# fmidev/RoadSurf

Hardware: AMD Instinct MI355X
Metric: point_timesteps_per_s (higher is better)
Workload: dtype f64

## Files before the change

### roadsurf_amd/csrc/rs_api.hip

```cpp
#include <hip/hip_runtime.h>
#include <atomic>
#include <cmath>
#include <cstdarg>
#include <cstdio>
#include <cstdlib>
#include <cstring>
#include <mutex>
#include <utility>
#include <vector>

#include "../../include/roadsurf.h"
#include "rs_kernels.h"
#include "rs_ens_table.hpp"
#include "rs_devutil.hpp"
#include <cstdint>
#include <algorithm>
#include "rs_consts_dev.h"
#include "rs_state.h"

static thread_local char g_err[512] = "";

static int set_err(const char *fmt, ...) {
  va_list ap;
  va_start(ap, fmt);
// ... 1266 lines not shown
  if (rs_read_div_mismatch(n, pl->stream) != hipSuccess) return -1;
  return which == 1 ? (int64_t)(n[1] + n[2]) : (int64_t)n[0];
}
int64_t rs_hip_div_mismatch_count(RsPlan *pl) { return div_mismatch(pl, 0); }
int64_t rs_hip_div_special_count(RsPlan *pl) { return div_mismatch(pl, 1); }
int rs_hip_div_samples(RsPlan *pl, double *out) {
  if (!pl || !out) return set_err("rs_hip_div_samples: bad arguments");
  HIP_OK(hipSetDevice(pl->device));
  HIP_OK(rs_read_div_samples(out, pl->stream));
  return 0;
}

int rs_hip_bl_stats(RsPlan *pl, int64_t *out) {
  if (!pl || !out) return set_err("rs_hip_bl_stats: bad arguments");
  HIP_OK(hipSetDevice(pl->device));
  unsigned long long v[56];
  HIP_OK(rs_read_bl_stats(v, pl->stream));
  for (int k = 0; k < 56; ++k) out[k] = (int64_t)v[k];
  return 0;
}

int rs_hip_division_mode(void) {
#if defined(RS_IEEE_DIV)
  return 0;
#elif defined(RS_DIV_CHECK)
  return 2;
#else
  return 1;
#endif
}

int rs_hip_test_math(RsPlan *pl, int32_t fn, int64_t n, const double *x, double *y) {
  if (!pl || !x || !y || n < 1 || fn < 0 || fn > 3) return set_err("rs_hip_test_math: bad arguments");
// ... 82 lines not shown
```

### roadsurf_amd/csrc/rs_consts_dev.h

```cpp
#pragma once
#include <cstdlib>
#include "../../include/roadsurf.h"

struct RsConstantsDev : RsConstants {
  double meltDen;
  double r_3600, r_3364, r_1000, r_IceMax, r_twoDT, r_DTSecs, r_meltDen, r_logUstar, r_logCond;
  int32_t bareFastOk;
  int32_t precFastOk;
  double chk[8];
  const double *relax_tab;
  const double *cpl_tab;
  double capDZF[RS_MAX_LAYERS + 2];
  double hs1F;
  double hcw[8];
  struct LayerRow {
    double capDZF, condDZ, DyC, dryCap, WCont, pad[3];
  } lk[RS_MAX_LAYERS + 2];
};

static inline void rs_consts_dev_fill(const RsConstants &c, RsConstantsDev &d) {
  static_cast<RsConstants &>(d) = c;
  d.meltDen = c.WatMHeat * c.WatDens;
  d.r_3600 = 1.0 / 3600.0;
  d.r_3364 = 1.0 / 3364.0;
  d.r_1000 = 1.0 / 1000.0;
  d.r_IceMax = 1.0 / 1.5;
  d.r_twoDT = 1.0 / c.twoDT;
  d.r_DTSecs = 1.0 / c.DTSecs;
  d.r_meltDen = 1.0 / d.meltDen;
  d.r_logUstar = 1.0 / c.logUstar;
  d.r_logCond = 1.0 / c.logCond;
  const float chk[8] = {100.0f, -0.1f, -90.0f, 120.0f, -1.0f, 4000.0f, 1000.0f, 500.0f};
  for (int i = 0; i < 8; ++i) d.chk[i] = (double)chk[i];
// ... 13 lines not shown
  }
  for (int j = 0; j < RS_MAX_LAYERS + 2; ++j) d.capDZF[j] = 0.0;
  d.hs1F = 0.0;
  for (int j = 1; j <= c.NLayers && j <= RS_MAX_LAYERS; ++j) {
    const volatile double chwt = 920.0 * 2100.0;
    const volatile double wc = c.WCont[j] * chwt;
    const volatile double vsh = c.dryCap[j] + wc;
    const volatile double den = c.DyC[j] * vsh;
    d.capDZF[j] = -(1.0 / den);
    d.lk[j].capDZF = d.capDZF[j];
    if (j == 1) {
      const volatile double num = vsh * c.HSfac1;
      d.hs1F = num / c.twoDT;
    }
  }
  d.bareFastOk = (c.MaxWatmms >= 0.0 && c.MaxSnowmms >= 0.0 && c.MaxIcemms >= 0.0 && c.MaxDepmms >= 0.0) ? 1 : 0;
  d.precFastOk = (c.MinPrecmm >= 0.0) ? 1 : 0;
}

static inline const char *rs_consts_domain_error(const RsConstants &c) {
  const double lo = 1e-30, hi = 1e30;
  auto pos = [&](double x) { return x > lo && x < hi; };
  auto mag = [&](double x) { return (x > lo && x < hi) || (x < -lo && x > -hi); };
  if (!pos(c.DTSecs) || !pos(c.twoDT)) return "DTSecs";
  if (!mag(c.logUstar)) return "logUstar = log(ZRefW/ZMom)";
  if (!mag(c.logCond)) return "logCond = log(ZRefT/ZHeat)";
  if (!(c.logMom > -hi && c.logMom < hi) || !(c.logHeat > -hi && c.logHeat < hi)) return "logMom/logHeat";
  if (!pos(c.VK_Const)) return "VK_Const";
  if (!pos(c.LVap) || !pos(c.LFus)) return "LVap/LFus";
  if (!pos(c.WatMHeat * c.WatDens)) return "WatMHeat*WatDens";
// ... 28 lines not shown
```

### roadsurf_amd/csrc/rs_kernels.hip

```cpp
#include <hip/hip_runtime.h>
#include <cstdlib>
#include "rs_physics.hpp"
#include "rs_state.h"
#include "rs_synth.h"
#include "rs_kernels.h"

#ifndef RS_CPL_WAVES
#define RS_CPL_WAVES 2
#endif
#ifndef RS_REGIME_WINDOW
#define RS_REGIME_WINDOW 30
#endif

namespace rs {

constexpr int kBlock = RS_BLOCK;

typedef RsConstantsDev __attribute__((address_space(4))) ConstsAS;
template <class Args>
__device__ __forceinline__ const ConstsAS &consts_of(Args a) {
  return *(const ConstsAS *)a->consts;
}

template <int NL, int NREG>
// ... 587 lines not shown
#endif
template <bool SCORE, bool A32>
__global__ void __launch_bounds__(kBlock, 4) step_kernel_hybrid(const StepArgs a) {
  __shared__ double math_lds[RS_MATH_LDS_DOUBLES];
  __shared__ double prof_lds[(15 - RS_HYBRID_REG) * kBlock];
  step_lanes<HybridProfile<15, RS_HYBRID_REG>, true, false, SCORE, false, false, A32>(a, math_lds, prof_lds);
}

template <bool FULL, bool DIAG = false>
__global__ void __launch_bounds__(kBlock, 4) step_kernel_lds(const StepArgs a) {
  extern __shared__ double lds[];
  __shared__ double math_lds[RS_MATH_LDS_DOUBLES];
  step_lanes<LdsProfile, FULL, false, true, false, false, false, DIAG>(a, math_lds, lds);
}

enum { PR_TAIR = 0, PR_VZ, PR_RHZ, PR_RAIN, PR_SNOW, PR_AVC, PR_EAIR, PR_SW, PR_LW, PR_OBS, PR_LEAN = PR_OBS, PR_FULL = PR_OBS + 1 };
template <int NPREP>
struct DuoMailT {
  double v[2][2][64];
  uint32_t failed[64];
  double prep[2][NPREP][64];
  uint32_t prep_bad[2][64];
};

template <bool FULL, bool SKYG = false, class Mail>
__device__ __forceinline__ void duo_put_prep(Mail &mail, int buf, uint32_t lane, const ForcingPrep &q) {
  double (*w)[64] = mail.prep[buf];
  w[PR_TAIR][lane] = q.tair; w[PR_VZ][lane] = q.vz; w[PR_RHZ][lane] = q.rhz; w[PR_RAIN][lane] = q.rain;
  w[PR_SNOW][lane] = q.snow;
  w[PR_AVC][lane] = q.AirHCap * q.AirDens;
  w[PR_EAIR][lane] = q.EAir;
  if (!SKYG) {
    w[PR_SW][lane] = q.sw;
    w[PR_LW][lane] = q.lw;
  }
  if (FULL) w[PR_OBS][lane] = q.tsurfobs;
  mail.prep_bad[buf][lane] = (q.bad ? 1u : 0u) | (q.night ? 2u : 0u) | (q.bad_rw ? 8u : 0u);
}
template <bool FULL, bool SKYG = false, class C, class Mail>
__device__ __forceinline__ ForcingPrep duo_get_prep(const C &c, const Mail &mail, int buf, uint32_t lane,
                                                    const uint32_t *skyfl = nullptr) {
  const double (*w)[64] = mail.prep[buf];
  ForcingPrep q;
  q.tair = w[PR_TAIR][lane]; q.vz = w[PR_VZ][lane]; q.rhz = w[PR_RHZ][lane]; q.rain = w[PR_RAIN][lane];
  q.snow = w[PR_SNOW][lane];
  const double AirVCap = w[PR_AVC][lane];
  q.AirVCap = AirVCap;
  q.EAir = w[PR_EAIR][lane]; q.sw = w[PR_SW][lane]; q.lw = w[PR_LW][lane];
  if (FULL) q.tsurfobs = w[PR_OBS][lane];
  uint32_t flags = mail.prep_bad[buf][lane];
  if (SKYG) flags |= skyfl[buf * 64 + lane];
  {
    const double fricN = c.TrfFricNgt, fricD = c.TrFfricDay;
    q.night = (flags & 2u) != 0u;
    q.trffric = q.night ? fricN : fricD;
  }
  q.PsychC = R4(0.1) * (R4(0.00063) * (q.tair + R4(273.15)) + R4(0.47496));
  q.den0 = AirVCap * (q.tair + R4(273.15));
  q.vkvz = c.VK_Const * q.vz;
  q.avk = AirVCap * c.VK_Const;
  q.bad = (flags & 1u) != 0u;
  q.stop = SKYG && (flags & 4u) != 0u;
  q.bad_rw = (flags & 8u) != 0u;
  return q;
}

__device__ __forceinline__ void duo_meet() { asm volatile("s_waitcnt lgkmcnt(0)\n\ts_barrier" ::: "memory"); }

template <int NL, bool SCORE, bool FULL = false, bool SKY = false, bool SKYG = false, bool OUTIDX = false,
          bool CPL = false, bool REPLAY = false>
__device__ __forceinline__ void duo_surface(const MathTab &mt, DuoMailT<FULL ? PR_FULL : PR_LEAN> &mail, const StepArgs &a,
                                            const uint32_t *skyfl = nullptr) {
// ... 1355 lines not shown
```

### roadsurf_amd/csrc/rs_math.hpp

```cpp
#pragma once
#include <hip/hip_runtime.h>
#include "rs_glibc_tables.h"

namespace rs {

static __constant__ uint64_t c_gl_exp_tab[256] = {0};
static __constant__ uint64_t c_gl_log_tab[256] = {0};

enum { RS_K_EXP_SHIFT, RS_K_EXP_C2, RS_K_EXP_C4, RS_K_LOG_A1, RS_K_LOG_A3, RS_K_LOG_B1,
       RS_K_LOG_B4, RS_K_LOG_B7, RS_K_COUNT };
static __constant__ uint64_t c_gl_coef[RS_K_COUNT] = {
    RS_GL_EXP_SHIFT, RS_GL_EXP_C2, RS_GL_EXP_C4, RS_GL_LOG_A1,
    RS_GL_LOG_A3,    RS_GL_LOG_B1, RS_GL_LOG_B4, RS_GL_LOG_B7};

enum { RS_S_EXP_INVLN2N, RS_S_EXP_NEGLN2HIN, RS_S_EXP_NEGLN2LON, RS_S_EXP_C3, RS_S_EXP_C5, RS_S_PAD0, RS_S_PAD1, RS_S_PAD2,
       RS_S_LOG_LN2HI, RS_S_LOG_A2, RS_S_LOG_LN2LO, RS_S_LOG_A4, RS_S_LOG_A0, RS_S_PAD3, RS_S_PAD4, RS_S_PAD5,
       RS_S_LOG_B2, RS_S_LOG_B5, RS_S_LOG_B8, RS_S_LOG_B3, RS_S_LOG_B6, RS_S_LOG_B9, RS_S_LOG_B10, RS_S_LOG_B0,
       RS_S_COUNT };
static __constant__ uint64_t c_gl_scoef[RS_S_COUNT] = {
    RS_GL_EXP_INVLN2N, RS_GL_EXP_NEGLN2HIN, RS_GL_EXP_NEGLN2LON, RS_GL_EXP_C3, RS_GL_EXP_C5, 0, 0, 0,
    RS_GL_LOG_LN2HI, RS_GL_LOG_A2, RS_GL_LOG_LN2LO, RS_GL_LOG_A4, RS_GL_LOG_A0, 0, 0, 0,
    RS_GL_LOG_B2, RS_GL_LOG_B5, RS_GL_LOG_B8, RS_GL_LOG_B3, RS_GL_LOG_B6, RS_GL_LOG_B9, RS_GL_LOG_B10, RS_GL_LOG_B0};
typedef const double __attribute__((address_space(4))) *MathCoef;

// ... 8 lines not shown

__device__ __forceinline__ MathTab fill_math_tables(double *lds) {
  uint64_t *w = reinterpret_cast<uint64_t *>(lds);
  for (int i = threadIdx.x; i < RS_MATH_LDS_DOUBLES; i += blockDim.x)
    w[i] = (i < 256) ? c_gl_exp_tab[i] : (i < 512) ? c_gl_log_tab[i - 256] : c_gl_coef[i - 512];
  MathTab t;
  t.expT = w;
  t.logT = lds + 256;
  t.K = lds + 512;
  t.S = (MathCoef)c_gl_scoef;
  asm volatile("" : "+s"(t.S));
  return t;
}

static __device__ unsigned long long g_div_mismatch[3] = {0ull, 0ull, 0ull};
#define RS_BL_NSTATS 56
static __device__ unsigned long long g_bl_stats[RS_BL_NSTATS];
#define RS_DIV_SAMPLES 64
static __device__ double g_div_samples[RS_DIV_SAMPLES][4];
__device__ __forceinline__ void div_check_note(double q, double f, double a = 0.0, double b = 0.0) {
  if (__double_as_longlong(q) == __double_as_longlong(f) || (q != q && f != f)) return;
  const bool special = !(__builtin_fabs(q) < __builtin_inf()) || !(__builtin_fabs(f) < __builtin_inf());
  const int kind = special ? 1 : (q == f ? 2 : 0);
  const unsigned long long k = atomicAdd(&g_div_mismatch[kind], 1ull);
  if (kind == 0 && k < RS_DIV_SAMPLES) {
    g_div_samples[k][0] = a;
    g_div_samples[k][1] = b;
    g_div_samples[k][2] = q;
    g_div_samples[k][3] = f;
  }
}
// ... 233 lines not shown
```

### roadsurf_amd/csrc/rs_physics.hpp

```cpp
#pragma once
#include <hip/hip_runtime.h>
#include "../../include/roadsurf.h"
#include "rs_math.hpp"
#include "rs_consts_dev.h"


#define RS_REAL double
#define RS_NS rs
#define RS_CONSTS RsConstantsDev __attribute__((address_space(4)))
#define RS_DIVC(a, b, rb) rs_div_u(a, b, c.rb)
#define RS_SECANT_DIV(a, b) ((a) / (b))
#define RS_PROFILE_PIN 1
#define RS_CPL_SLOTS(c) true
#define RS_CPL_DECAY_TABLE 1
#define RS_GEN_PREFETCH 1
#define RS_GEN_FP64_FEATURES 1
#define RS_INIT_KERNEL init_kernel
#define RS_INIT_ANCHOR R4(-99.9)
#define RS_INIT_ZERO_TAIL 1
#define RS_BL_GUARD 1
#define RS_MELTDEN c.meltDen
#define RS_BARE_FAST(c) ((c).bareFastOk != 0)
#define RS_PREC_FAST(c) ((c).precFastOk != 0)
#define RS_CHK(c, i, lit) ((c).chk[i])
// ... 2 lines not shown
#define RS_FROZEN_TABLE 1
#endif
#ifndef RS_NO_LAYER_ROWS
#define RS_LK(c, j, name) ((c).lk[j].name)
#else
#define RS_LK(c, j, name) ((c).name[j])
#endif
#ifndef RS_NO_HCW_TABLE
#define RS_HCW_TABLE 1
#endif
#define RS_STAB_UPPER(x) rs_min_one(x)
#ifndef RS_NO_DRY_TAIL_SKIP
#define RS_DRY_TAIL 1
#if !defined(RS_NO_DRY_ESURF_SKIP) && !defined(RS_EXP_SURFACE_LIGHT) && !defined(RS_EXP_PIPE1)
#define RS_DRY_ESURF 1
#endif
#endif
#include "rs_physics_body.inc"
#undef RS_DRY_TAIL
#undef RS_DRY_ESURF
#undef RS_STAB_UPPER
#undef RS_FROZEN_TABLE
#undef RS_HCW_TABLE
#undef RS_LK
#undef RS_NS
#undef RS_CONSTS
#undef RS_BL_GUARD
#undef RS_MELTDEN
#undef RS_BARE_FAST
#undef RS_PREC_FAST
// ... 4 lines not shown
```

### roadsurf_amd/csrc/rs_physics_body.inc

```
namespace RS_NS {

struct Scalars {
  RS_REAL tnw1, tnw2;
  RS_REAL tsurf;
  RS_REAL wat, snow, ice, ice2, dep;
  RS_REAL q2melt, t4melt, albedo;
  RS_REAL tair_end, vz_end, rh_end;
  bool verycold, failed;
};

struct Forcing {
  RS_REAL tair, tdew, vz, rhz, prec, sw, lw, tsurfobs, depth;
  int32_t phase, hour;
};

template <class Prof>
__device__ __forceinline__ RS_REAL temp_at_depth(const RS_CONSTS &c, const Prof &T, RS_REAL tbot,
                                                RS_REAL depth) {
  const int N = T.nlayers();
  if (rs_fabs(depth - R4(0.0)) < R4(0.00001)) return T.get(1);
  if (depth > c.ZDpth[N + 1]) return tbot;
  RS_REAL r = 0.0;
  bool found = false;
#pragma unroll
// ... 93 lines not shown
  v.vkvz = c.VK_Const * vz;
  v.avk = AirVCap * c.VK_Const;
#ifdef RS_EXP_STAB_CHAIN
  v.kinv = rs_div((RS_REAL)1.0, v.den0 * (v.vkvz * v.vkvz * v.vkvz));
#endif
  x.PSIM = R4(0.0);
  x.PSIH = R4(0.0);
  x.BLCond = 0.0;
}

__device__ __forceinline__ RS_REAL bl_stab_num(const RS_CONSTS &c) {
  return -c.VK_Const * c.ZRefT * c.Grav;
}

template <bool IEEE = false>
__device__ __forceinline__ bool bl_iteration(const RS_CONSTS &c, const MathTab &mt,
                                             const BlInv &v, BlVar &x, int j, RS_REAL stab_num,
                                             bool *unstable = nullptr) {
  const RS_REAL ConvLim = R4(0.001);
  const RS_REAL BLCond_Old = x.BLCond;
  RS_REAL UStar;
  if (!IEEE && j == 1) {
    UStar = RS_DIVC(v.vkvz, c.logUstar, r_logUstar);
    x.BLCond = RS_DIVC(v.avk * UStar, c.logCond, r_logCond);
  } else {
    UStar = rs_dvb<IEEE>(v.vkvz, c.logUstar + x.PSIM);
    x.BLCond = rs_dvb<IEEE>(v.avk * UStar, c.logCond + x.PSIH);
  }
#ifdef RS_EXP_STAB_CHAIN
  const RS_REAL a_ = (!IEEE && j == 1) ? c.logUstar : c.logUstar + x.PSIM;
  RS_REAL Stab = (stab_num * x.BLCond * v.dT) * ((a_ * a_ * a_) * v.kinv);
#else
  RS_REAL Stab = rs_dvb<IEEE>(stab_num * x.BLCond * v.dT, v.den0 * (UStar * UStar * UStar));
#endif
#ifndef RS_STAB_UPPER
  if (Stab > 1) Stab = 1;
#endif
  if (Stab > 0) {
#ifdef RS_STAB_UPPER
    x.PSIH = R4(4.7) * RS_STAB_UPPER(Stab);
#else
    x.PSIH = R4(4.7) * Stab;
#endif
    x.PSIM = x.PSIH;
  } else {
    x.PSIH = R4(-2.0) * rs_log(mt, (R4(1.0) + rs_sq<IEEE>(R4(1.0) - R4(16.0) * Stab)) / R4(2.0));
    x.PSIM = R4(0.6) * x.PSIH;
    if (unstable) *unstable = true;
  }
  return (j >= 5) && (rs_fabs(x.BLCond - BLCond_Old) < ConvLim);
}

#ifdef RS_DRY_TAIL
__device__ __forceinline__ bool dry_tail_signs(RS_REAL wat, RS_REAL raNum, RS_REAL raDen) {
  return (wat <= R4(0.0)) && (raNum > R4(0.0)) && rs_is_pos_finite(raDen);
}
__device__ __forceinline__ bool dry_tail_le(bool signs, RS_REAL N, RS_REAL PsychC) {
  return signs && rs_is_pos_normal(N) && (PsychC > R4(0.0)) && (PsychC < R4(1.0));
}
__device__ __forceinline__ bool dry_tail_warm(bool signs, RS_REAL tsurf, RS_REAL tair, RS_REAL EAir) {
  return signs && (tair > R4(-100.0)) && (tsurf < R4(100.0)) && (tsurf >= tair + R4(0.01)) && (EAir == EAir);
}
#ifdef RS_BL_STATS
__device__ __forceinline__ void dry_tail_count(bool le_dry, bool warm) {
  const unsigned long long act = __builtin_amdgcn_ballot_w64(true), m1 = __builtin_amdgcn_ballot_w64(le_dry),
                           m2 = __builtin_amdgcn_ballot_w64(warm);
  if ((unsigned long long)__builtin_ctzll(act) == (unsigned long long)(threadIdx.x & 63u)) {
    if (m1 == act) atomicAdd(&rs::g_bl_stats[49], 1ull);
    atomicAdd(&rs::g_bl_stats[50], (unsigned long long)__builtin_popcountll(m1));
    if (m2 == act) atomicAdd(&rs::g_bl_stats[51], 1ull);
    atomicAdd(&rs::g_bl_stats[52], (unsigned long long)__builtin_popcountll(m2));
  }
}
#endif
#endif

template <bool IEEE = false>
__device__ __forceinline__ void bl_finish(const RS_CONSTS &c, const MathTab &mt, const BlAux &a,
                                          const BlVar &x, RS_REAL tsurf, RS_REAL tair, RS_REAL vz,
                                          RS_REAL rhz, RS_REAL wat, RS_REAL &le, RS_REAL &evap) {
#ifdef RS_DRY_TAIL
  const RS_REAL raNum = (c.logMom + x.PSIM) * (c.logHeat + x.PSIH), raDen = c.VK_Const * c.VK_Const * vz;
  const RS_REAL aa = (tair < 0) ? R4(21.875) : R4(17.269);
  const RS_REAL ba = (tair < 0) ? R4(265.5) : R4(237.3);
  const RS_REAL ESat = R4(0.61078) * rs_exp(mt, rs_dv<IEEE>(aa * tair, tair + ba));
  const RS_REAL EAir = rs_min_num_one(R4(0.01) * rhz) * ESat;
  const bool signs = dry_tail_signs(wat, raNum, raDen);
#ifdef RS_DRY_ESURF
  if (!IEEE && rs_wave_all(dry_tail_warm(signs, tsurf, tair, EAir))) {
    le = R4(0.0);
    evap = R4(0.0);
    return;
  }
#endif
  const RS_REAL as = (tsurf < 0) ? R4(21.875) : R4(17.269);
  const RS_REAL bs = (tsurf < 0) ? R4(265.5) : R4(237.3);
  const RS_REAL ESurf = R4(0.61078) * rs_exp(mt, rs_dv<IEEE>(as * tsurf, tsurf + bs));
  const RS_REAL N = a.AirDens * a.AirHCap * (ESurf - EAir);
  if (!IEEE && rs_wave_all(dry_tail_le(signs, N, a.PsychC))) {
    le = R4(0.0);
    evap = R4(0.0);
    return;
  }
// ... 383 lines not shown
                                                    int32_t phase, int32_t hour,
                                                    const CouplingInputs &cp = CouplingInputs()) {
  Fluxes fx;
  fluxes_pre(c, mt, s, tair, vz, rhz, prec_ts, phase, hour, fx);
  boundary_layer<TRIPS>(c, mt, s.tsurf, tair, vz, rhz, s.wat, fx.blcond, fx.le, fx.evap, fx.trips);
  fluxes_post(c, s, sw, lw, cp, fx);
  return fx;
}

struct ForcingPrep {
  RS_REAL tair, vz, rhz;
  RS_REAL rain, snow;
  RS_REAL trffric;
  RS_REAL AirDens, AirHCap, PsychC, den0, vkvz, avk;
  RS_REAL AirVCap = 0;
  RS_REAL EAir;
  RS_REAL sw, lw;
  bool bad;
  bool night = false;
  bool stop = false;
  bool bad_rw = false;
  RS_REAL tsurfobs = R4(-9999.9);
};

__device__ __forceinline__ bool check_values_forcing(const RS_CONSTS &c, const Forcing &f) {
  const RS_REAL hi100 = rs_fmax(f.tair, f.vz);
  const RS_REAL lo01 = rs_fmin(rs_fmin(f.rhz, f.sw), rs_fmin(f.lw, f.prec));
  return (hi100 > RS_CHK(c, 0, R4(100.0))) | (lo01 < RS_CHK(c, 1, R4(-0.1))) |
         (f.tair < RS_CHK(c, 2, R4(-90.0))) | (f.rhz > RS_CHK(c, 3, R4(120.0))) |
         (f.vz < RS_CHK(c, 4, R4(-1.0))) | (f.sw > RS_CHK(c, 5, R4(4000.0))) |
         (f.lw > RS_CHK(c, 6, R4(1000.0))) | (f.prec > RS_CHK(c, 7, R4(500.0)));
// ... 3 lines not shown
  return rs_fabs(tsurf) > RS_CHK(c, 0, R4(100.0));
}

__device__ __forceinline__ RS_REAL forcing_prep_head(const RS_CONSTS &c, const Forcing &f, int32_t i,
                                                     bool checked, bool has_tdew, bool &bad) {
  RS_REAL vz = f.vz;
  if (i == 1 && vz < R4(0.4)) vz = R4(0.4);
  bad = false;
  if (checked) {
    Forcing chk = f;
    chk.vz = vz;
    bad = check_values_forcing(c, chk);
    if (has_tdew) bad = bad | (f.tdew < -90) | (f.tdew > R4(100.0));
  }
  return vz;
}

template <bool NIGHT_U = false>
__device__ __forceinline__ ForcingPrep forcing_prep_tail(const RS_CONSTS &c, const MathTab &mt, const Forcing &f,
                                                         RS_REAL tair, RS_REAL vz, RS_REAL rhz, bool bad,
                                                         bool night_u = false) {
  ForcingPrep q;
  RS_REAL prec_ts = RS_DIVC(f.prec, (RS_REAL)3600.0, r_3600) * c.DTSecs;
  q.bad = bad;
  {
    Scalars z;
    z.wat = R4(0.0);
    z.snow = R4(0.0);
#ifdef RS_BL_STATS
    {
// ... 16 lines not shown
  q.trffric = night ? fricN : fricD;
  q.night = night;
  if (vz < calm) vz = calm;
  q.tair = tair;
  q.vz = vz;
  q.rhz = rhz;
  const RS_REAL TaK = tair + R4(273.15);
  q.AirDens = rs_dv<false>(R4(100000.0), R4(287.05) * TaK);
  const RS_REAL dK = (TaK - R4(250.0)) * (TaK - R4(250.0));
  q.AirHCap = R4(1005.0) + RS_DIVC(dK, R4(3364.), r_3364);
  const RS_REAL AirVCap = q.AirHCap * q.AirDens;
  q.PsychC = R4(0.1) * (R4(0.00063) * TaK + R4(0.47496));
  q.den0 = AirVCap * (tair + R4(273.15));
  q.vkvz = c.VK_Const * vz;
  q.avk = AirVCap * c.VK_Const;
  const RS_REAL aa = (tair < 0) ? R4(21.875) : R4(17.269);
  const RS_REAL ba = (tair < 0) ? R4(265.5) : R4(237.3);
  const RS_REAL ESat = R4(0.61078) * rs_exp(mt, rs_dv<false>(aa * tair, tair + ba));
  q.EAir = rs_min_num_one(R4(0.01) * rhz) * ESat;
  q.sw = f.sw;
  q.lw = f.lw;
  return q;
}

template <bool NIGHT_U = false>
__device__ __forceinline__ ForcingPrep forcing_prep(const RS_CONSTS &c, const MathTab &mt, const Forcing &f,
                                                    int32_t i, bool checked, bool night_u = false) {
  bool bad;
  const RS_REAL vz = forcing_prep_head(c, f, i, checked, false, bad);
  return forcing_prep_tail<NIGHT_U>(c, mt, f, f.tair, vz, f.rhz, bad, night_u);
}

template <int TRIPS = 1>
__device__ __forceinline__ Fluxes model_step_fluxes_prepped(const RS_CONSTS &c, const MathTab &mt,
                                                            Scalars &s, const ForcingPrep &q,
                                                            const CouplingInputs &cp = CouplingInputs()) {
  Fluxes fx;
  s.wat = s.wat + q.rain;
  s.snow = s.snow + q.snow;
  fx.trffric = q.trffric;
  BlInv v;
  BlVar x;
  BlAux a;
  a.PsychC = q.PsychC;
#ifndef RS_DRY_TAIL
  const RS_REAL WatDen = R4(-0.0050) * s.tsurf * s.tsurf + R4(0.0079) * s.tsurf + R4(1000.0028);
#endif
  v.dT = s.tsurf - q.tair;
  v.den0 = q.den0;
  v.vkvz = q.vkvz;
  v.avk = q.avk;
#ifdef RS_EXP_STAB_CHAIN
  v.kinv = rs_div((RS_REAL)1.0, v.den0 * (v.vkvz * v.vkvz * v.vkvz));
#endif
  x.PSIM = R4(0.0);
  x.PSIH = R4(0.0);
  x.BLCond = 0.0;
  const RS_REAL stab_num = bl_stab_num(c);
  int j = 1;
  bool unstable = false;
#ifdef RS_BL_STATS
  {
    const unsigned long long act = __builtin_amdgcn_ballot_w64(true);
    const bool first = (unsigned long long)__builtin_ctzll(act) == (unsigned long long)(threadIdx.x & 63u);
    if (first) {
      atomicAdd(&rs::g_bl_stats[0], 1ull);
      atomicAdd(&rs::g_bl_stats[1], (unsigned long long)__builtin_popcountll(act));
    }
    for (; j <= RS_BL_MAXIT; ++j) {
      const RS_REAL h0 = x.PSIH;
      const bool done = bl_iteration<false>(c, mt, v, x, j, stab_num, TRIPS == 1 ? &unstable : nullptr);
      {
        const bool uns = !(x.PSIH > R4(0.0)), far = x.PSIH < R4(-0.1254);
        const unsigned long long mu = __builtin_amdgcn_ballot_w64(uns), mf = __builtin_amdgcn_ballot_w64(far),
                                 ma = __builtin_amdgcn_ballot_w64(true);
        if ((unsigned long long)__builtin_ctzll(ma) == (unsigned long long)(threadIdx.x & 63u)) {
          atomicAdd(&rs::g_bl_stats[19], 1ull);
          atomicAdd(&rs::g_bl_stats[48], (unsigned long long)__builtin_popcountll(ma));
          atomicAdd(&rs::g_bl_stats[46], (unsigned long long)__builtin_popcountll(mu));
          atomicAdd(&rs::g_bl_stats[47], (unsigned long long)__builtin_popcountll(mf));
          if (mu) atomicAdd(&rs::g_bl_stats[20], 1ull);
          if (mf && (mu & ~mf)) atomicAdd(&rs::g_bl_stats[21], 1ull);
          if (mu && (ma & ~mu)) atomicAdd(&rs::g_bl_stats[22], 1ull);
          if (mf) atomicAdd(&rs::g_bl_stats[23], 1ull);
        }
      }
      if (j >= 2 && j <= 4) {
        const bool same = __double_as_longlong((double)h0) == __double_as_longlong((double)x.PSIH);
        const unsigned long long ms = __builtin_amdgcn_ballot_w64(same);
        if (first) {
          if (ms == act) atomicAdd(&rs::g_bl_stats[j], 1ull);
          atomicAdd(&rs::g_bl_stats[3 + j], (unsigned long long)__builtin_popcountll(ms));
        }
      }
      if (done) break;
    }
    {
      const int trips = j > RS_BL_MAXIT ? RS_BL_MAXIT : j;
      int wmax = trips, wsum = trips;
      for (int o = 32; o > 0; o >>= 1) {
        const int other = __shfl_xor(wmax, o, 64);
        wmax = other > wmax ? other : wmax;
        wsum += __shfl_xor(wsum, o, 64);
      }
      auto bin = [](int t) { return t <= 8 ? t - 5 : t <= 12 ? 4 : t <= 20 ? 5 : t < 40 ? 6 : 7; };
      for (int b = 0; b < 8; ++b) {
        const unsigned long long mb = __builtin_amdgcn_ballot_w64(bin(trips) == b);
        if (first && mb) atomicAdd(&rs::g_bl_stats[32 + b], (unsigned long long)__builtin_popcountll(mb));
      }
      {
        const int nh = __builtin_popcountll(__builtin_amdgcn_ballot_w64(trips > 20));
        if (first && nh > 0) atomicAdd(&rs::g_bl_stats[40 + (nh == 1 ? 0 : nh <= 3 ? 1 : nh <= 7 ? 2 : nh <= 15 ? 3 : nh <= 31 ? 4 : 5)], 1ull);
      }
      if (first) {
        atomicAdd(&rs::g_bl_stats[9], (unsigned long long)wsum);
        atomicAdd(&rs::g_bl_stats[8], (unsigned long long)wmax);
        atomicAdd(&rs::g_bl_stats[24 + bin(wmax)], 1ull);
      }
    }
  }
#else
#ifdef RS_EXP_PIPE1
  const RS_REAL as_ = (s.tsurf < 0) ? R4(21.875) : R4(17.269);
  const RS_REAL bs_ = (s.tsurf < 0) ? R4(265.5) : R4(237.3);
  const RS_REAL ESurf_ = R4(0.61078) * rs_exp(mt, rs_dv<false>(as_ * s.tsurf, s.tsurf + bs_));
  (void)bl_iteration<false>(c, mt, v, x, 1, stab_num, TRIPS == 1 ? &unstable : nullptr);
  j = 2;
#endif
  for (; j <= RS_BL_MAXIT; ++j)
    if (bl_iteration<false>(c, mt, v, x, j, stab_num, TRIPS == 1 ? &unstable : nullptr)) break;
#endif
  fx.trips = TRIPS == 1 ? j + (unstable ? 64 : 0) : TRIPS == 2 ? (j > RS_BL_MAXIT ? RS_BL_MAXIT : j) : 5;
  fx.blcond = x.BLCond;
  do {
    const RS_REAL raNum = (c.logMom + x.PSIM) * (c.logHeat + x.PSIH), raDen = c.VK_Const * c.VK_Const * q.vz;
#ifdef RS_DRY_TAIL
    const bool signs = dry_tail_signs(s.wat, raNum, raDen);
#endif
#ifdef RS_DRY_ESURF
    const bool warm = dry_tail_warm(signs, s.tsurf, q.tair, q.EAir);
#ifndef RS_BL_STATS
    if (rs_wave_all(warm)) {
      fx.le = R4(0.0);
      fx.evap = R4(0.0);
      break;
    }
#endif
#endif
    const RS_REAL as = (s.tsurf < 0) ? R4(21.875) : R4(17.269);
    const RS_REAL bs = (s.tsurf < 0) ? R4(265.5) : R4(237.3);
#ifdef RS_EXP_SURFACE_LIGHT
    const RS_REAL ESurf = R4(0.61078) + (as + bs) * R4(0.0001) * s.tsurf;
#elif defined(RS_EXP_PIPE1)
    const RS_REAL ESurf = ESurf_;
    (void)as; (void)bs;
#else
    const RS_REAL ESurf = R4(0.61078) * rs_exp(mt, rs_dv<false>(as * s.tsurf, s.tsurf + bs));
#endif
    const RS_REAL N = q.AirVCap * (ESurf - q.EAir);
#ifdef RS_DRY_TAIL
    const bool le_dry = dry_tail_le(signs, N, a.PsychC);
#if defined(RS_BL_STATS) && defined(RS_DRY_ESURF)
    dry_tail_count(le_dry, warm);
#endif
    if (rs_wave_all(le_dry)) {
      fx.le = R4(0.0);
      fx.evap = R4(0.0);
      break;
    }
    asm volatile("");
    const RS_REAL WatDen = R4(-0.0050) * s.tsurf * s.tsurf + R4(0.0079) * s.tsurf + R4(1000.0028);
#endif
    RS_REAL RAero = rs_dvb<false>(raNum, raDen);
    if (RAero > R4(30.0)) RAero = R4(30.);
// ... 5 lines not shown
      fx.le = R4(0.0);
      fx.evap = R4(0.0);
    }
  } while (false);
#if RS_BL_GUARD && !defined(RS_IEEE_DIV) && !defined(RS_DIV_CHECK) && !defined(RS_NO_BL_GUARD) && !defined(RS_BL_FIXUP)
  if (!(rs_fabs(fx.blcond) < __builtin_inf()) || !(rs_fabs(fx.le) < __builtin_inf())) {
    const BlOut o = boundary_layer_ieee(&c, mt.expT, mt.logT, mt.K, s.tsurf, q.tair, q.vz, q.rhz, s.wat);
    fx.blcond = o.blcond;
    fx.le = o.le;
    fx.evap = o.evap;
  }
#endif
  fluxes_post(c, s, q.sw, q.lw, cp, fx);
  return fx;
}

__device__ __forceinline__ RS_REAL layer_step(const RS_CONSTS &c, int j, RS_REAL tj, RS_REAL tstale,
                                              RS_REAL tnext, RS_REAL &Gprev, RS_REAL *hs1) {
#ifdef RS_FROZEN_TABLE
  RS_REAL ncap;
  const unsigned long long thawed = __builtin_amdgcn_ballot_w64(tstale >= 0);
#ifdef RS_EXP_SURFACE_LIGHT
  if (j <= 2) {
    ncap = -RS_LK(c, j, capDZF);
    if (hs1) *hs1 = c.hs1F;
  } else
#endif
  if (thawed == 0ull) {
    ncap = -RS_LK(c, j, capDZF);
    if (hs1) *hs1 = c.hs1F;
// ... 74 lines not shown
```

Baseline: 26.35 billion.

## Skip final boundary-layer stability update and defer air vapour pressure to surface flux

Splits the boundary-layer iteration into a pass and a stability-arm step so the last arm (with its exp/log) can be skipped when a whole wave is dry, warm and stable beyond a host-precomputed safe threshold. Air vapour pressure (an exp and a divide) is no longer computed during forcing prep. It is recomputed only when the latent-heat numerator is actually needed, which also drops one prep mailbox slot. PsychC is computed lazily. Correctness relies on the stabSafe bound and the dry/warm predicates exactly matching the zero-flux outcome, and the added wave-uniform branches may cost some divergence.

```diff
diff --git a/roadsurf_amd/csrc/rs_api.hip b/roadsurf_amd/csrc/rs_api.hip
--- a/roadsurf_amd/csrc/rs_api.hip
+++ b/roadsurf_amd/csrc/rs_api.hip
@@ -1304,9 +1304,9 @@
 int rs_hip_bl_stats(RsPlan *pl, int64_t *out) {
   if (!pl || !out) return set_err("rs_hip_bl_stats: bad arguments");
   HIP_OK(hipSetDevice(pl->device));
-  unsigned long long v[56];
+  unsigned long long v[57];
   HIP_OK(rs_read_bl_stats(v, pl->stream));
-  for (int k = 0; k < 56; ++k) out[k] = (int64_t)v[k];
+  for (int k = 0; k < 57; ++k) out[k] = (int64_t)v[k];
   return 0;
 }
 
diff --git a/roadsurf_amd/csrc/rs_consts_dev.h b/roadsurf_amd/csrc/rs_consts_dev.h
--- a/roadsurf_amd/csrc/rs_consts_dev.h
+++ b/roadsurf_amd/csrc/rs_consts_dev.h
@@ -1,4 +1,5 @@
 #pragma once
+#include <cmath>
 #include <cstdlib>
 #include "../../include/roadsurf.h"
 
@@ -16,7 +17,15 @@
   struct LayerRow {
     double capDZF, condDZ, DyC, dryCap, WCont, pad[3];
   } lk[RS_MAX_LAYERS + 2];
+  double stabSafe;
 };
+
+static inline double rs_stab_safe(double logMom, double logHeat) {
+  if (!(logMom > 0.0 && logMom < HUGE_VAL && logHeat > 0.0 && logHeat < HUGE_VAL)) return NAN;
+  const double psih = std::fmin(logHeat / 2.0, logMom / 1.2);
+  const double sq = 2.0 * std::exp(psih / 2.0) - 1.0;
+  return (1.0 - sq * sq) / 16.0;
+}
 
 static inline void rs_consts_dev_fill(const RsConstants &c, RsConstantsDev &d) {
   static_cast<RsConstants &>(d) = c;
@@ -60,6 +69,7 @@
       d.hs1F = num / c.twoDT;
     }
   }
+  d.stabSafe = rs_stab_safe(c.logMom, c.logHeat);
   d.bareFastOk = (c.MaxWatmms >= 0.0 && c.MaxSnowmms >= 0.0 && c.MaxIcemms >= 0.0 && c.MaxDepmms >= 0.0) ? 1 : 0;
   d.precFastOk = (c.MinPrecmm >= 0.0) ? 1 : 0;
 }
diff --git a/roadsurf_amd/csrc/rs_kernels.hip b/roadsurf_amd/csrc/rs_kernels.hip
--- a/roadsurf_amd/csrc/rs_kernels.hip
+++ b/roadsurf_amd/csrc/rs_kernels.hip
@@ -625,7 +625,11 @@
   step_lanes<LdsProfile, FULL, false, true, false, false, false, DIAG>(a, math_lds, lds);
 }
 
+#ifdef RS_EAIR_SURFACE
+enum { PR_TAIR = 0, PR_VZ, PR_RHZ, PR_RAIN, PR_SNOW, PR_AVC, PR_SW, PR_LW, PR_OBS, PR_LEAN = PR_OBS, PR_FULL = PR_OBS + 1 };
+#else
 enum { PR_TAIR = 0, PR_VZ, PR_RHZ, PR_RAIN, PR_SNOW, PR_AVC, PR_EAIR, PR_SW, PR_LW, PR_OBS, PR_LEAN = PR_OBS, PR_FULL = PR_OBS + 1 };
+#endif
 template <int NPREP>
 struct DuoMailT {
   double v[2][2][64];
@@ -640,7 +644,9 @@
   w[PR_TAIR][lane] = q.tair; w[PR_VZ][lane] = q.vz; w[PR_RHZ][lane] = q.rhz; w[PR_RAIN][lane] = q.rain;
   w[PR_SNOW][lane] = q.snow;
   w[PR_AVC][lane] = q.AirHCap * q.AirDens;
+#ifndef RS_EAIR_SURFACE
   w[PR_EAIR][lane] = q.EAir;
+#endif
   if (!SKYG) {
     w[PR_SW][lane] = q.sw;
     w[PR_LW][lane] = q.lw;
@@ -657,7 +663,10 @@
   q.snow = w[PR_SNOW][lane];
   const double AirVCap = w[PR_AVC][lane];
   q.AirVCap = AirVCap;
-  q.EAir = w[PR_EAIR][lane]; q.sw = w[PR_SW][lane]; q.lw = w[PR_LW][lane];
+#ifndef RS_EAIR_SURFACE
+  q.EAir = w[PR_EAIR][lane];
+#endif
+  q.sw = w[PR_SW][lane]; q.lw = w[PR_LW][lane];
   if (FULL) q.tsurfobs = w[PR_OBS][lane];
   uint32_t flags = mail.prep_bad[buf][lane];
   if (SKYG) flags |= skyfl[buf * 64 + lane];
@@ -666,7 +675,9 @@
     q.night = (flags & 2u) != 0u;
     q.trffric = q.night ? fricN : fricD;
   }
+#ifndef RS_BL_LAST
   q.PsychC = R4(0.1) * (R4(0.00063) * (q.tair + R4(273.15)) + R4(0.47496));
+#endif
   q.den0 = AirVCap * (q.tair + R4(273.15));
   q.vkvz = c.VK_Const * q.vz;
   q.avk = AirVCap * c.VK_Const;
diff --git a/roadsurf_amd/csrc/rs_math.hpp b/roadsurf_amd/csrc/rs_math.hpp
--- a/roadsurf_amd/csrc/rs_math.hpp
+++ b/roadsurf_amd/csrc/rs_math.hpp
@@ -46,7 +46,7 @@
 }
 
 static __device__ unsigned long long g_div_mismatch[3] = {0ull, 0ull, 0ull};
-#define RS_BL_NSTATS 56
+#define RS_BL_NSTATS 57
 static __device__ unsigned long long g_bl_stats[RS_BL_NSTATS];
 #define RS_DIV_SAMPLES 64
 static __device__ double g_div_samples[RS_DIV_SAMPLES][4];
diff --git a/roadsurf_amd/csrc/rs_physics.hpp b/roadsurf_amd/csrc/rs_physics.hpp
--- a/roadsurf_amd/csrc/rs_physics.hpp
+++ b/roadsurf_amd/csrc/rs_physics.hpp
@@ -40,6 +40,12 @@
 #define RS_DRY_TAIL 1
 #if !defined(RS_NO_DRY_ESURF_SKIP) && !defined(RS_EXP_SURFACE_LIGHT) && !defined(RS_EXP_PIPE1)
 #define RS_DRY_ESURF 1
+#if !defined(RS_NO_BL_LAST_SKIP) && !defined(RS_EXP_STAB_CHAIN)
+#define RS_BL_LAST 1
+#endif
+#ifndef RS_NO_EAIR_SURFACE
+#define RS_EAIR_SURFACE 1
+#endif
 #endif
 #endif
 #include "rs_physics_body.inc"
diff --git a/roadsurf_amd/csrc/rs_physics_body.inc b/roadsurf_amd/csrc/rs_physics_body.inc
--- a/roadsurf_amd/csrc/rs_physics_body.inc
+++ b/roadsurf_amd/csrc/rs_physics_body.inc
@@ -131,9 +131,8 @@
 }
 
 template <bool IEEE = false>
-__device__ __forceinline__ bool bl_iteration(const RS_CONSTS &c, const MathTab &mt,
-                                             const BlInv &v, BlVar &x, int j, RS_REAL stab_num,
-                                             bool *unstable = nullptr) {
+__device__ __forceinline__ bool bl_pass(const RS_CONSTS &c, const BlInv &v, BlVar &x, int j, RS_REAL stab_num,
+                                        RS_REAL &Stab) {
   const RS_REAL ConvLim = R4(0.001);
   const RS_REAL BLCond_Old = x.BLCond;
   RS_REAL UStar;
@@ -146,10 +145,15 @@
   }
 #ifdef RS_EXP_STAB_CHAIN
   const RS_REAL a_ = (!IEEE && j == 1) ? c.logUstar : c.logUstar + x.PSIM;
-  RS_REAL Stab = (stab_num * x.BLCond * v.dT) * ((a_ * a_ * a_) * v.kinv);
-#else
-  RS_REAL Stab = rs_dvb<IEEE>(stab_num * x.BLCond * v.dT, v.den0 * (UStar * UStar * UStar));
-#endif
+  Stab = (stab_num * x.BLCond * v.dT) * ((a_ * a_ * a_) * v.kinv);
+#else
+  Stab = rs_dvb<IEEE>(stab_num * x.BLCond * v.dT, v.den0 * (UStar * UStar * UStar));
+#endif
+  return (j >= 5) && (rs_fabs(x.BLCond - BLCond_Old) < ConvLim);
+}
+
+template <bool IEEE = false>
+__device__ __forceinline__ void bl_arm(const MathTab &mt, RS_REAL Stab, BlVar &x, bool *unstable = nullptr) {
 #ifndef RS_STAB_UPPER
   if (Stab > 1) Stab = 1;
 #endif
@@ -165,10 +169,26 @@
     x.PSIM = R4(0.6) * x.PSIH;
     if (unstable) *unstable = true;
   }
-  return (j >= 5) && (rs_fabs(x.BLCond - BLCond_Old) < ConvLim);
+}
+
+template <bool IEEE = false>
+__device__ __forceinline__ bool bl_iteration(const RS_CONSTS &c, const MathTab &mt,
+                                             const BlInv &v, BlVar &x, int j, RS_REAL stab_num,
+                                             bool *unstable = nullptr) {
+  RS_REAL Stab;
+  const bool done = bl_pass<IEEE>(c, v, x, j, stab_num, Stab);
+  bl_arm<IEEE>(mt, Stab, x, unstable);
+  return done;
 }
 
 #ifdef RS_DRY_TAIL
+__device__ __forceinline__ bool dry_tail_dry(RS_REAL wat, RS_REAL raDen) {
+  return (wat <= R4(0.0)) && rs_is_pos_finite(raDen);
+}
+__device__ __forceinline__ bool dry_tail_warm_t(RS_REAL tsurf, RS_REAL tair) {
+  return (tair > R4(-100.0)) && (tsurf < R4(100.0)) && (tsurf >= tair + R4(0.01));
+}
+__device__ __forceinline__ bool dry_tail_psychc(RS_REAL PsychC) { return (PsychC > R4(0.0)) && (PsychC < R4(1.0)); }
 __device__ __forceinline__ bool dry_tail_signs(RS_REAL wat, RS_REAL raNum, RS_REAL raDen) {
   return (wat <= R4(0.0)) && (raNum > R4(0.0)) && rs_is_pos_finite(raDen);
 }
@@ -198,12 +218,19 @@
                                           RS_REAL rhz, RS_REAL wat, RS_REAL &le, RS_REAL &evap) {
 #ifdef RS_DRY_TAIL
   const RS_REAL raNum = (c.logMom + x.PSIM) * (c.logHeat + x.PSIH), raDen = c.VK_Const * c.VK_Const * vz;
+  const bool signs = dry_tail_signs(wat, raNum, raDen);
+#if defined(RS_DRY_ESURF) && defined(RS_EAIR_SURFACE)
+  if (!IEEE && rs_wave_all(signs && dry_tail_warm_t(tsurf, tair))) {
+    le = R4(0.0);
+    evap = R4(0.0);
+    return;
+  }
+#endif
   const RS_REAL aa = (tair < 0) ? R4(21.875) : R4(17.269);
   const RS_REAL ba = (tair < 0) ? R4(265.5) : R4(237.3);
   const RS_REAL ESat = R4(0.61078) * rs_exp(mt, rs_dv<IEEE>(aa * tair, tair + ba));
   const RS_REAL EAir = rs_min_num_one(R4(0.01) * rhz) * ESat;
-  const bool signs = dry_tail_signs(wat, raNum, raDen);
-#ifdef RS_DRY_ESURF
+#if defined(RS_DRY_ESURF) && !defined(RS_EAIR_SURFACE)
   if (!IEEE && rs_wave_all(dry_tail_warm(signs, tsurf, tair, EAir))) {
     le = R4(0.0);
     evap = R4(0.0);
@@ -617,7 +644,9 @@
   RS_REAL trffric;
   RS_REAL AirDens, AirHCap, PsychC, den0, vkvz, avk;
   RS_REAL AirVCap = 0;
+#ifndef RS_EAIR_SURFACE
   RS_REAL EAir;
+#endif
   RS_REAL sw, lw;
   bool bad;
   bool night = false;
@@ -651,6 +680,13 @@
     if (has_tdew) bad = bad | (f.tdew < -90) | (f.tdew > R4(100.0));
   }
   return vz;
+}
+
+__device__ __forceinline__ RS_REAL air_vapour_pressure(const MathTab &mt, RS_REAL tair, RS_REAL rhz) {
+  const RS_REAL aa = (tair < 0) ? R4(21.875) : R4(17.269);
+  const RS_REAL ba = (tair < 0) ? R4(265.5) : R4(237.3);
+  const RS_REAL ESat = R4(0.61078) * rs_exp(mt, rs_dv<false>(aa * tair, tair + ba));
+  return rs_min_num_one(R4(0.01) * rhz) * ESat;
 }
 
 template <bool NIGHT_U = false>
@@ -697,10 +733,9 @@
   q.den0 = AirVCap * (tair + R4(273.15));
   q.vkvz = c.VK_Const * vz;
   q.avk = AirVCap * c.VK_Const;
-  const RS_REAL aa = (tair < 0) ? R4(21.875) : R4(17.269);
-  const RS_REAL ba = (tair < 0) ? R4(265.5) : R4(237.3);
-  const RS_REAL ESat = R4(0.61078) * rs_exp(mt, rs_dv<false>(aa * tair, tair + ba));
-  q.EAir = rs_min_num_one(R4(0.01) * rhz) * ESat;
+#ifndef RS_EAIR_SURFACE
+  q.EAir = air_vapour_pressure(mt, tair, rhz);
+#endif
   q.sw = f.sw;
   q.lw = f.lw;
   return q;
@@ -714,6 +749,202 @@
   return forcing_prep_tail<NIGHT_U>(c, mt, f, f.tair, vz, f.rhz, bad, night_u);
 }
 
+#ifdef RS_BL_STATS
+struct BlStatsStep {
+  unsigned long long act;
+  bool first;
+};
+__device__ __forceinline__ BlStatsStep bl_stats_step() {
+  const unsigned long long act = __builtin_amdgcn_ballot_w64(true);
+  const bool first = (unsigned long long)__builtin_ctzll(act) == (unsigned long long)(threadIdx.x & 63u);
+  if (first) {
+    atomicAdd(&rs::g_bl_stats[0], 1ull);
+    atomicAdd(&rs::g_bl_stats[1], (unsigned long long)__builtin_popcountll(act));
+  }
+  return BlStatsStep{act, first};
+}
+__device__ __forceinline__ void bl_stats_pass(const BlStatsStep &st, int j, RS_REAL h0, const BlVar &x) {
+  const unsigned long long act = st.act;
+  const bool first = st.first;
+  {
+    const bool uns = !(x.PSIH > R4(0.0)), far = x.PSIH < R4(-0.1254);
+    const unsigned long long mu = __builtin_amdgcn_ballot_w64(uns), mf = __builtin_amdgcn_ballot_w64(far),
+                             ma = __builtin_amdgcn_ballot_w64(true);
+    if ((unsigned long long)__builtin_ctzll(ma) == (unsigned long long)(threadIdx.x & 63u)) {
+      atomicAdd(&rs::g_bl_stats[19], 1ull);
+      atomicAdd(&rs::g_bl_stats[48], (unsigned long long)__builtin_popcountll(ma));
+      atomicAdd(&rs::g_bl_stats[46], (unsigned long long)__builtin_popcountll(mu));
+      atomicAdd(&rs::g_bl_stats[47], (unsigned long long)__builtin_popcountll(mf));
+      if (mu) atomicAdd(&rs::g_bl_stats[20], 1ull);
+      if (mf && (mu & ~mf)) atomicAdd(&rs::g_bl_stats[21], 1ull);
+      if (mu && (ma & ~mu)) atomicAdd(&rs::g_bl_stats[22], 1ull);
+      if (mf) atomicAdd(&rs::g_bl_stats[23], 1ull);
+    }
+  }
+  if (j >= 2 && j <= 4) {
+    const bool same = __double_as_longlong((double)h0) == __double_as_longlong((double)x.PSIH);
+    const unsigned long long ms = __builtin_amdgcn_ballot_w64(same);
+    if (first) {
+      if (ms == act) atomicAdd(&rs::g_bl_stats[j], 1ull);
+      atomicAdd(&rs::g_bl_stats[3 + j], (unsigned long long)__builtin_popcountll(ms));
+    }
+  }
+}
+__device__ __forceinline__ void bl_stats_trips(const BlStatsStep &st, int j) {
+  const bool first = st.first;
+  {
+    const int trips = j > RS_BL_MAXIT ? RS_BL_MAXIT : j;
+    int wmax = trips, wsum = trips;
+    for (int o = 32; o > 0; o >>= 1) {
+      const int other = __shfl_xor(wmax, o, 64);
+      wmax = other > wmax ? other : wmax;
+      wsum += __shfl_xor(wsum, o, 64);
+    }
+    auto bin = [](int t) { return t <= 8 ? t - 5 : t <= 12 ? 4 : t <= 20 ? 5 : t < 40 ? 6 : 7; };
+    for (int b = 0; b < 8; ++b) {
+      const unsigned long long mb = __builtin_amdgcn_ballot_w64(bin(trips) == b);
+      if (first && mb) atomicAdd(&rs::g_bl_stats[32 + b], (unsigned long long)__builtin_popcountll(mb));
+    }
+    {
+      const int nh = __builtin_popcountll(__builtin_amdgcn_ballot_w64(trips > 20));
+      if (first && nh > 0) atomicAdd(&rs::g_bl_stats[40 + (nh == 1 ? 0 : nh <= 3 ? 1 : nh <= 7 ? 2 : nh <= 15 ? 3 : nh <= 31 ? 4 : 5)], 1ull);
+    }
+    if (first) {
+      atomicAdd(&rs::g_bl_stats[9], (unsigned long long)wsum);
+      atomicAdd(&rs::g_bl_stats[8], (unsigned long long)wmax);
+      atomicAdd(&rs::g_bl_stats[24 + bin(wmax)], 1ull);
+    }
+  }
+}
+#endif
+
+#ifdef RS_BL_LAST
+__device__ __forceinline__ RS_REAL le_numerator(const MathTab &mt, RS_REAL tsurf, const ForcingPrep &q) {
+  const RS_REAL as = (tsurf < 0) ? R4(21.875) : R4(17.269);
+  const RS_REAL bs = (tsurf < 0) ? R4(265.5) : R4(237.3);
+  const RS_REAL ESurf = R4(0.61078) * rs_exp(mt, rs_dv<false>(as * tsurf, tsurf + bs));
+#ifdef RS_EAIR_SURFACE
+  const RS_REAL EAir = air_vapour_pressure(mt, q.tair, q.rhz);
+#else
+  const RS_REAL EAir = q.EAir;
+#endif
+  return q.AirVCap * (ESurf - EAir);
+}
+__device__ __forceinline__ RS_REAL psychrometric(RS_REAL tair) {
+  return R4(0.1) * (R4(0.00063) * (tair + R4(273.15)) + R4(0.47496));
+}
+#ifdef RS_BL_STATS
+__device__ __forceinline__ void bl_last_count(bool dead, bool skip, bool all_warm, RS_REAL Stab) {
+  const unsigned long long act = __builtin_amdgcn_ballot_w64(true), mu = __builtin_amdgcn_ballot_w64(!(Stab > R4(0.0)));
+  if ((unsigned long long)__builtin_ctzll(act) == (unsigned long long)(threadIdx.x & 63u)) {
+    if (dead) atomicAdd(&rs::g_bl_stats[53], 1ull);
+    if (skip) atomicAdd(&rs::g_bl_stats[54], 1ull);
+    if (skip && mu) atomicAdd(&rs::g_bl_stats[55], 1ull);
+    if (all_warm) atomicAdd(&rs::g_bl_stats[56], 1ull);
+  }
+}
+#endif
+
+template <int TRIPS = 1>
+__device__ __forceinline__ Fluxes model_step_fluxes_prepped(const RS_CONSTS &c, const MathTab &mt,
+                                                            Scalars &s, const ForcingPrep &q,
+                                                            const CouplingInputs &cp = CouplingInputs()) {
+  Fluxes fx;
+  s.wat = s.wat + q.rain;
+  s.snow = s.snow + q.snow;
+  fx.trffric = q.trffric;
+  BlInv v;
+  BlVar x;
+  v.dT = s.tsurf - q.tair;
+  v.den0 = q.den0;
+  v.vkvz = q.vkvz;
+  v.avk = q.avk;
+  x.PSIM = R4(0.0);
+  x.PSIH = R4(0.0);
+  x.BLCond = 0.0;
+  const RS_REAL stab_num = bl_stab_num(c);
+  const RS_REAL raDen = c.VK_Const * c.VK_Const * q.vz;
+  const bool dry = dry_tail_dry(s.wat, raDen);
+  const bool warm = dry && dry_tail_warm_t(s.tsurf, q.tair);
+  const bool all_warm = rs_wave_all(warm);
+  RS_REAL N = R4(0.0);
+  bool dead = true;
+#ifdef RS_BL_STATS
+  const bool need_n = true;
+#else
+  const bool need_n = !all_warm;
+#endif
+  if (need_n) {
+    asm volatile("");
+    N = le_numerator(mt, s.tsurf, q);
+    dead = rs_wave_all(warm || (dry && rs_is_pos_normal(N) && dry_tail_psychc(psychrometric(q.tair))));
+  }
+  RS_REAL Stab = R4(0.0);
+  int j = 1;
+  bool unstable = false;
+#ifdef RS_BL_STATS
+  {
+    const BlStatsStep st = bl_stats_step();
+    for (; j <= RS_BL_MAXIT; ++j) {
+      const RS_REAL h0 = x.PSIH;
+      const bool done = bl_pass<false>(c, v, x, j, stab_num, Stab);
+      bl_arm<false>(mt, Stab, x, TRIPS == 1 ? &unstable : nullptr);
+      bl_stats_pass(st, j, h0, x);
+      if (done) break;
+    }
+    bl_stats_trips(st, j);
+  }
+#else
+  for (; j <= RS_BL_MAXIT; ++j) {
+    if (j >= 2) bl_arm<false>(mt, Stab, x, TRIPS == 1 ? &unstable : nullptr);
+    if (bl_pass<false>(c, v, x, j, stab_num, Stab)) break;
+  }
+  if (TRIPS == 1 && !(Stab > R4(0.0))) unstable = true;
+#endif
+  fx.trips = TRIPS == 1 ? j + (unstable ? 64 : 0) : TRIPS == 2 ? (j > RS_BL_MAXIT ? RS_BL_MAXIT : j) : 5;
+  fx.blcond = x.BLCond;
+  const bool skip = dead && rs_wave_all(Stab > c.stabSafe);
+#ifdef RS_BL_STATS
+  {
+    const RS_REAL raNum = (c.logMom + x.PSIM) * (c.logHeat + x.PSIH);
+    dry_tail_count(dry_tail_le(dry_tail_signs(s.wat, raNum, raDen), N, psychrometric(q.tair)), warm && (raNum > R4(0.0)));
+    bl_last_count(dead, skip, all_warm, Stab);
+  }
+#endif
+  if (skip) {
+    fx.le = R4(0.0);
+    fx.evap = R4(0.0);
+  } else {
+    asm volatile("");
+#ifndef RS_BL_STATS
+    bl_arm<false>(mt, Stab, x);
+#endif
+    const RS_REAL raNum = (c.logMom + x.PSIM) * (c.logHeat + x.PSIH);
+    if (!need_n) N = le_numerator(mt, s.tsurf, q);
+    const RS_REAL WatDen = R4(-0.0050) * s.tsurf * s.tsurf + R4(0.0079) * s.tsurf + R4(1000.0028);
+    RS_REAL RAero = rs_dvb<false>(raNum, raDen);
+    if (RAero > R4(30.0)) RAero = R4(30.);
+    fx.le = rs_dvb<false>(N, psychrometric(q.tair) * RAero);
+    const RS_REAL lvap = c.LVap, lfus = c.LFus;
+    const RS_REAL lat = (s.tsurf >= R4(0.0)) ? lvap : lfus;
+    fx.evap = rs_dvb<false>(fx.le, lat * WatDen) * R4(1000.0) * c.DTSecs;
+    if ((fx.le > R4(0.0)) && (s.wat <= R4(0.0))) {
+      fx.le = R4(0.0);
+      fx.evap = R4(0.0);
+    }
+  }
+#if RS_BL_GUARD && !defined(RS_IEEE_DIV) && !defined(RS_DIV_CHECK) && !defined(RS_NO_BL_GUARD) && !defined(RS_BL_FIXUP)
+  if (!(rs_fabs(fx.blcond) < __builtin_inf()) || !(rs_fabs(fx.le) < __builtin_inf())) {
+    const BlOut o = boundary_layer_ieee(&c, mt.expT, mt.logT, mt.K, s.tsurf, q.tair, q.vz, q.rhz, s.wat);
+    fx.blcond = o.blcond;
+    fx.le = o.le;
+    fx.evap = o.evap;
+  }
+#endif
+  fluxes_post(c, s, q.sw, q.lw, cp, fx);
+  return fx;
+}
+#else
 template <int TRIPS = 1>
 __device__ __forceinline__ Fluxes model_step_fluxes_prepped(const RS_CONSTS &c, const MathTab &mt,
                                                             Scalars &s, const ForcingPrep &q,
@@ -744,63 +975,14 @@
   bool unstable = false;
 #ifdef RS_BL_STATS
   {
-    const unsigned long long act = __builtin_amdgcn_ballot_w64(true);
-    const bool first = (unsigned long long)__builtin_ctzll(act) == (unsigned long long)(threadIdx.x & 63u);
-    if (first) {
-      atomicAdd(&rs::g_bl_stats[0], 1ull);
-      atomicAdd(&rs::g_bl_stats[1], (unsigned long long)__builtin_popcountll(act));
-    }
+    const BlStatsStep st = bl_stats_step();
     for (; j <= RS_BL_MAXIT; ++j) {
       const RS_REAL h0 = x.PSIH;
       const bool done = bl_iteration<false>(c, mt, v, x, j, stab_num, TRIPS == 1 ? &unstable : nullptr);
-      {
-        const bool uns = !(x.PSIH > R4(0.0)), far = x.PSIH < R4(-0.1254);
-        const unsigned long long mu = __builtin_amdgcn_ballot_w64(uns), mf = __builtin_amdgcn_ballot_w64(far),
-                                 ma = __builtin_amdgcn_ballot_w64(true);
-        if ((unsigned long long)__builtin_ctzll(ma) == (unsigned long long)(threadIdx.x & 63u)) {
-          atomicAdd(&rs::g_bl_stats[19], 1ull);
-          atomicAdd(&rs::g_bl_stats[48], (unsigned long long)__builtin_popcountll(ma));
-          atomicAdd(&rs::g_bl_stats[46], (unsigned long long)__builtin_popcountll(mu));
-          atomicAdd(&rs::g_bl_stats[47], (unsigned long long)__builtin_popcountll(mf));
-          if (mu) atomicAdd(&rs::g_bl_stats[20], 1ull);
-          if (mf && (mu & ~mf)) atomicAdd(&rs::g_bl_stats[21], 1ull);
-          if (mu && (ma & ~mu)) atomicAdd(&rs::g_bl_stats[22], 1ull);
-          if (mf) atomicAdd(&rs::g_bl_stats[23], 1ull);
-        }
-      }
-      if (j >= 2 && j <= 4) {
-        const bool same = __double_as_longlong((double)h0) == __double_as_longlong((double)x.PSIH);
-        const unsigned long long ms = __builtin_amdgcn_ballot_w64(same);
-        if (first) {
-          if (ms == act) atomicAdd(&rs::g_bl_stats[j], 1ull);
-          atomicAdd(&rs::g_bl_stats[3 + j], (unsigned long long)__builtin_popcountll(ms));
-        }
-      }
+      bl_stats_pass(st, j, h0, x);
       if (done) break;
     }
-    {
-      const int trips = j > RS_BL_MAXIT ? RS_BL_MAXIT : j;
-      int wmax = trips, wsum = trips;
-      for (int o = 32; o > 0; o >>= 1) {
-        const int other = __shfl_xor(wmax, o, 64);
-        wmax = other > wmax ? other : wmax;
-        wsum += __shfl_xor(wsum, o, 64);
-      }
-      auto bin = [](int t) { return t <= 8 ? t - 5 : t <= 12 ? 4 : t <= 20 ? 5 : t < 40 ? 6 : 7; };
-      for (int b = 0; b < 8; ++b) {
-        const unsigned long long mb = __builtin_amdgcn_ballot_w64(bin(trips) == b);
-        if (first && mb) atomicAdd(&rs::g_bl_stats[32 + b], (unsigned long long)__builtin_popcountll(mb));
-      }
-      {
-        const int nh = __builtin_popcountll(__builtin_amdgcn_ballot_w64(trips > 20));
-        if (first && nh > 0) atomicAdd(&rs::g_bl_stats[40 + (nh == 1 ? 0 : nh <= 3 ? 1 : nh <= 7 ? 2 : nh <= 15 ? 3 : nh <= 31 ? 4 : 5)], 1ull);
-      }
-      if (first) {
-        atomicAdd(&rs::g_bl_stats[9], (unsigned long long)wsum);
-        atomicAdd(&rs::g_bl_stats[8], (unsigned long long)wmax);
-        atomicAdd(&rs::g_bl_stats[24 + bin(wmax)], 1ull);
-      }
-    }
+    bl_stats_trips(st, j);
   }
 #else
 #ifdef RS_EXP_PIPE1
@@ -821,7 +1003,11 @@
     const bool signs = dry_tail_signs(s.wat, raNum, raDen);
 #endif
 #ifdef RS_DRY_ESURF
+#ifdef RS_EAIR_SURFACE
+    const bool warm = signs && dry_tail_warm_t(s.tsurf, q.tair);
+#else
     const bool warm = dry_tail_warm(signs, s.tsurf, q.tair, q.EAir);
+#endif
 #ifndef RS_BL_STATS
     if (rs_wave_all(warm)) {
       fx.le = R4(0.0);
@@ -840,7 +1026,12 @@
 #else
     const RS_REAL ESurf = R4(0.61078) * rs_exp(mt, rs_dv<false>(as * s.tsurf, s.tsurf + bs));
 #endif
-    const RS_REAL N = q.AirVCap * (ESurf - q.EAir);
+#ifdef RS_EAIR_SURFACE
+    const RS_REAL EAir = air_vapour_pressure(mt, q.tair, q.rhz);
+#else
+    const RS_REAL EAir = q.EAir;
+#endif
+    const RS_REAL N = q.AirVCap * (ESurf - EAir);
 #ifdef RS_DRY_TAIL
     const bool le_dry = dry_tail_le(signs, N, a.PsychC);
 #if defined(RS_BL_STATS) && defined(RS_DRY_ESURF)
@@ -876,6 +1067,7 @@
   fluxes_post(c, s, q.sw, q.lw, cp, fx);
   return fx;
 }
+#endif
 
 __device__ __forceinline__ RS_REAL layer_step(const RS_CONSTS &c, int j, RS_REAL tj, RS_REAL tstale,
                                               RS_REAL tnext, RS_REAL &Gprev, RS_REAL *hs1) {
```

Result: faster. 27.21 billion (median of 6 runs) (+3.3%).
